# decisionforce/CoPO

Hardware: AMD Instinct MI355X
Metric: agent-env-steps/sec (sim+learn), Intersection 40-agent (higher is better)
Workload: dtype f32; 1 GPU; CoPO Intersection, 40 agent slots x 256 scenes per GPU, fp32 (BASELINE configs[1]); rollout_steps=8, sgd_minibatch_size_per_rank=512, num_sgd_iter=5, lcf_num_iters=5, parallelism=dp1, hip_graphs=True, policy_init=reference population copo_inter (tests/golden, weights as data)

## Files before the change

copo_amd/_capi.py:

```python
import ctypes as C
import os

_HERE = os.path.dirname(os.path.abspath(__file__))
LIB_PATH = os.path.join(_HERE, "lib", "libcopo_hip.so")
try:
    from . import _libsel as _sel
    if getattr(_sel, "PATH", None):
        LIB_PATH = _sel.PATH
except ImportError:
    pass

from ._abi import *

LCF_STATS_DOUBLES = 8 + 6 * 2048

F_ACTED, F_DONE, F_ARRIVE, F_CRASH, F_OUT, F_MAXSTEP, F_SPAWNED, F_ENV_RESET = (1 << i for i in range(8))
I_VELOCITY, I_STEERING, I_ACCELERATION, I_STEP_REWARD, I_COST, I_EPISODE_LENGTH, I_EPISODE_REWARD, \
    I_ROUTE_COMPLETION = range(8)

ERR_NAMES = {0: "COPO_OK", -1: "COPO_ERR_NULL", -2: "COPO_ERR_DIM", -3: "COPO_ERR_DEVICE", -4: "COPO_ERR_STATE",
             -5: "COPO_ERR_CONFIG"}


class CopoError(RuntimeError):
# ... 11 lines not shown
    _fields_ = [
        ("mb", C.c_int32), ("hidden", C.c_int32), ("act_dim", C.c_int32), ("n_value_heads", C.c_int32),
        ("pack_width", C.c_int32), ("col_actions", C.c_int32), ("col_logp", C.c_int32), ("col_dist", C.c_int32),
        ("col_adv", C.c_int32), ("col_meta_adv", C.c_int32), ("col_vpred", C.c_int32 * 3), ("col_vtarget", C.c_int32 * 3),
        ("use_kl", C.c_int32), ("old_value_loss", C.c_int32), ("operand_dtype", C.c_int32), ("reserved0", C.c_int32),
        ("clip_param", C.c_float), ("vf_clip_param", C.c_float), ("vf_loss_coeff", C.c_float), ("entropy_coeff", C.c_float),
        ("lr", C.c_float), ("beta1", C.c_float), ("beta2", C.c_float), ("eps", C.c_float),
        ("pol", NetLayout), ("val", NetLayout * 3), ("n_params", C.c_int64),
    ]


HEAD_PPO, HEAD_META_NEW, HEAD_META_OLD = 0, 1, 2
OPERAND_F32, OPERAND_BF16 = 0, 1
PPO_STATS = 8
META_DOT_PARTIALS = 8192

_SIGS = {
    "copo_ppo_workspace_floats": (C.c_int64, [C.POINTER(PpoCfg)]),
    "copo_ppo_fused_step_f32": (C.c_int, [C.POINTER(PpoCfg)] + [C.c_void_p] * 14 + [C.c_int32, C.c_int32, C.c_void_p,
                                                                                   C.c_int32, C.c_void_p, C.c_void_p]),
    "copo_gather_rows_f32": (C.c_int, [C.POINTER(C.c_void_p), C.POINTER(C.c_void_p), C.POINTER(C.c_int32), C.c_int32, C.c_void_p,
                                       C.c_int64, C.c_void_p]),
    "copo_pack_columns_f32": (C.c_int, [C.POINTER(C.c_void_p), C.POINTER(C.c_int32), C.c_int32, C.c_int64, C.c_void_p, C.c_void_p]),
    "copo_dp_workspace_bytes": (C.c_int64, [C.POINTER(PpoCfg), C.c_int32]),
    "copo_ppo_fused_step_dp_f32": (C.c_int, [C.POINTER(PpoCfg)] + [C.c_void_p] * 13 + [C.c_void_p, C.c_int32, C.c_void_p,
                                                                                      C.POINTER(C.c_void_p), C.c_int32, C.c_int32, C.c_void_p]),
    "copo_dp_status": (C.c_int, [C.c_void_p, C.POINTER(PpoCfg), C.c_int32, C.c_void_p]),
    "copo_transpose_weights_f32": (C.c_int, [C.POINTER(PpoCfg), C.c_void_p, C.c_void_p, C.c_void_p]),
    "copo_mlp_forward_f32": (C.c_int, [C.POINTER(PpoCfg)] + [C.c_void_p] * 4 + [C.c_int64, C.c_int32, C.c_int32] +
                             [C.c_void_p] * 7),
# ... 20 lines not shown
    "copo_fault_obs": (C.c_int, [C.c_void_p] * 2 + [C.c_int32] * 5 + [C.c_void_p] * 2 + [C.c_int32] * 2 + [C.c_void_p] * 2 + [C.c_int32, C.c_void_p,
                                 C.c_uint64, C.c_void_p]),
    "copo_fault_act": (C.c_int, [C.c_void_p] * 3 + [C.c_int32] * 2 + [C.c_void_p] * 2 + [C.c_int32] * 2 + [C.c_void_p] * 2 + [C.c_int32, C.c_void_p,
                                 C.c_uint64, C.c_void_p]),
    "copo_adam_step_f32": (C.c_int, [C.POINTER(PpoCfg)] + [C.c_void_p] * 4 + [C.c_int64] + [C.c_void_p] * 5),
    "copo_meta_grads_f32": (C.c_int, [C.POINTER(PpoCfg)] + [C.c_void_p] * 15),
    "copo_meta_lcf_f64": (C.c_int, [C.c_void_p, C.c_int32, C.c_int32, C.c_int32] + [C.c_void_p] * 4 + [C.c_int32] +
                          [C.c_void_p] * 5),
    "copo_meta_finish_f64": (C.c_int, [C.c_void_p, C.c_void_p, C.c_int64, C.c_void_p, C.c_void_p, C.c_void_p, C.c_void_p, C.c_double,
                                       C.c_void_p, C.c_void_p, C.c_void_p, C.c_void_p, C.c_int32, C.c_void_p]),
    "copo_meta_step_f64": (C.c_int, [C.POINTER(PpoCfg)] + [C.c_void_p] * 13 + [C.c_int32, C.c_int32] + [C.c_void_p] * 5 +
                           [C.c_double, C.c_void_p, C.c_void_p, C.c_int32, C.c_void_p]),
    "copo_episode_metrics": (C.c_int, [C.c_void_p, C.c_void_p, C.c_void_p, C.c_int64, C.c_void_p, C.c_void_p]),
    "copo_plan_epoch": (C.c_int, [C.c_void_p, C.c_void_p, C.c_void_p, C.c_int64, C.c_int32, C.c_int32, C.c_void_p, C.c_int32] +
                        [C.c_void_p] * 5),
    "copo_meta_fold_len": (C.c_int64, [C.POINTER(PpoCfg)]),
    "copo_meta_batch_workspace_floats": (C.c_int64, [C.POINTER(PpoCfg), C.c_int32]),
    "copo_meta_batch_grads_f32": (C.c_int, [C.POINTER(PpoCfg)] + [C.c_void_p] * 8 + [C.c_int32, C.c_int64, C.c_int32] + [C.c_void_p] * 4),
    "copo_meta_batch_dot_f64": (C.c_int, [C.c_void_p, C.c_int64, C.c_int32, C.c_void_p, C.c_void_p, C.c_void_p, C.c_void_p]),
    "copo_meta_rows_workspace_floats": (C.c_int64, [C.POINTER(PpoCfg), C.c_int64]),
    "copo_meta_rows_f32": (C.c_int, [C.POINTER(PpoCfg)] + [C.c_void_p] * 4 + [C.c_int64] + [C.c_void_p] * 3),
    "copo_meta_batch_wgrads_f32": (C.c_int, [C.POINTER(PpoCfg)] + [C.c_void_p] * 5 + [C.c_int64] + [C.c_void_p] * 2 +
                                   [C.c_int32, C.c_int64, C.c_int32] + [C.c_void_p] * 4),
    "copo_meta_rowstat_f32": (C.c_int, [C.POINTER(PpoCfg)] + [C.c_void_p] * 4 + [C.c_int64, C.c_int32, C.c_void_p, C.c_void_p]),
    "copo_meta_batch_lcf_f64": (C.c_int, [C.c_void_p, C.c_int32, C.c_int32, C.c_int32, C.c_void_p, C.c_void_p, C.c_int32] +
                                [C.c_void_p] * 3 + [C.c_int32, C.c_int32] + [C.c_void_p] * 5 + [C.c_double, C.c_void_p, C.c_int32, C.c_int32, C.c_int32, C.c_void_p, C.c_void_p]),
    "copo_version": (C.c_int, []),
    "copo_build_info": (C.c_char_p, []),
    "copo_last_error": (C.c_char_p, []),
    "copo_sim_create": (C.c_int, [C.POINTER(SimCfg), C.c_int, C.POINTER(C.c_void_p)]),
# ... 82 lines not shown
    "copo_recorder_count": (C.c_int, [C.c_void_p, C.POINTER(C.c_int64), C.c_void_p]),
    "copo_recorder_read": (C.c_int, [C.c_void_p, C.c_int32, C.c_int32, C.c_void_p, C.c_void_p]),
    "copo_recorder_episodes": (C.c_int, [C.c_void_p, C.c_void_p, C.c_void_p]),
    "copo_recorder_clear": (C.c_int, [C.c_void_p, C.c_void_p]),
    "copo_recorder_reset": (C.c_int, [C.c_void_p, C.c_void_p]),
    "copo_recorder_destroy": (C.c_int, [C.c_void_p]),
    "copo_neighbours_f32": (C.c_int, [C.c_void_p, C.c_void_p, C.c_void_p, C.c_int32, C.c_int32, C.c_int32, C.c_float,
                                      C.c_float, C.c_void_p, C.c_void_p, C.c_void_p, C.c_void_p, C.c_void_p,
                                      C.c_void_p, C.c_void_p]),
    "copo_gae3_f32": (C.c_int, [C.c_void_p, C.c_void_p, C.c_void_p, C.c_int32, C.c_int32, C.c_int32,
                                C.POINTER(C.c_double), C.c_double, C.c_void_p, C.c_void_p, C.c_void_p]),
    "copo_cc_fuse_mf_f32": (C.c_int, [C.c_void_p] * 5 + [C.c_int32] * 6 + [C.c_void_p, C.c_void_p]),
    "copo_cc_fuse_concat_f32": (C.c_int, [C.c_void_p] * 5 + [C.c_int32] * 7 + [C.c_void_p, C.c_void_p]),
    "copo_lcf_mix_partial_f32": (C.c_int, [C.c_void_p] * 5 + [C.c_int64, C.c_void_p, C.c_void_p, C.c_void_p]),
    "copo_lcf_mix_apply_f32": (C.c_int, [C.c_void_p] * 3 + [C.c_int64, C.c_void_p, C.c_void_p, C.c_void_p, C.c_void_p]),
    "copo_peer_workspace_bytes": (C.c_int64, [C.c_int64, C.c_int32]),
    "copo_peer_alloc": (C.c_int, [C.c_int64, C.POINTER(C.c_void_p)]),
    "copo_peer_free": (C.c_int, [C.c_void_p]),
    "copo_ipc_export": (C.c_int, [C.c_void_p, C.c_char_p]),
    "copo_ipc_open": (C.c_int, [C.c_char_p, C.POINTER(C.c_void_p)]),
    "copo_ipc_close": (C.c_int, [C.c_void_p]),
    "copo_peer_allreduce_sum_f32": (C.c_int, [C.POINTER(C.c_void_p), C.c_int64, C.c_int32, C.c_int32, C.c_void_p]),
    "copo_peer_status": (C.c_int, [C.c_void_p, C.c_int64, C.c_int32, C.c_void_p]),
    "copo_debug_peer_allreduce_all_ranks": (C.c_int, [C.POINTER(C.c_void_p), C.c_int64, C.c_int32, C.c_void_p]),
    "copo_debug_rowpass_stamps": (C.c_int, [C.c_void_p]),
    "copo_debug_wg_times": (C.c_int, [C.c_void_p]),
    "copo_debug_learner_plan": (C.c_int, [C.POINTER(PpoCfg), C.c_int32, C.c_int32, C.c_int64] + [C.c_int32] * 5 + [C.c_void_p, C.c_int32]),
    "copo_debug_learner_kernel": (C.c_char_p, [C.c_int32, C.POINTER(C.c_int32), C.POINTER(C.c_int32)]),
}

# ... 40 lines not shown
```

copo_amd/csrc/capi.hip:

```cpp
#include <cstdarg>
#include <cstdio>
#include <cstring>
#include <new>
#include <algorithm>
#include <vector>
#include <cmath>

#include "capi_common.h"
#include "seat_common.h"
#include "fault_common.h"

using namespace copo;

static thread_local char g_err[512] = "";

int copo::fail(int code, const char* fmt, ...) {
    va_list ap;
    va_start(ap, fmt);
    vsnprintf(g_err, sizeof(g_err), fmt, ap);
    va_end(ap);
    return code;
}

extern "C" int copo_version(void) { return COPO_ABI_VERSION; }
// ... 503 lines not shown
extern "C" int copo_lcf_mix_partial_f32(const float* adv, const float* nei_adv, const float* glob_adv, const float* lcf,
                                        const uint8_t* valid, int64_t B, float* mixed, double* stats, void* stream) {
    if (!adv || !nei_adv || !glob_adv || !lcf || !mixed || !stats)
        return fail(COPO_ERR_NULL, "copo_lcf_mix_partial_f32: NULL argument");
    if (B < 0) return fail(COPO_ERR_DIM, "copo_lcf_mix_partial_f32: B=%lld", (long long)B);
    HIP_TRY(launch_lcf_mix_partial(adv, nei_adv, glob_adv, lcf, valid, B, mixed, stats, static_cast<hipStream_t>(stream)));
    return COPO_OK;
}

extern "C" int copo_lcf_mix_apply_f32(const float* mixed, const float* glob_adv, const uint8_t* valid, int64_t B,
                                      const double* stats, float* norm_adv, float* glob_adv_std, void* stream) {
    if (!mixed || !glob_adv || !stats || !norm_adv || !glob_adv_std)
        return fail(COPO_ERR_NULL, "copo_lcf_mix_apply_f32: NULL argument");
    if (B < 0) return fail(COPO_ERR_DIM, "copo_lcf_mix_apply_f32: B=%lld", (long long)B);
    if (B == 0) return COPO_OK;
    HIP_TRY(launch_lcf_mix_apply(mixed, glob_adv, valid, B, stats, norm_adv, glob_adv_std, static_cast<hipStream_t>(stream)));
    return COPO_OK;
}
```

copo_amd/csrc/learn_kernels.hip:

```cpp
#include <string.h>

#include "sim_common.h"

namespace copo {

struct Gae3Args {
    double gamma[4];
    double lam;
};

__global__ void __launch_bounds__(256) gae3_kernel(const float* __restrict__ rew, const float* __restrict__ val,
                                                   const uint8_t* __restrict__ flags, int T, int M, int heads,
                                                   Gae3Args a, float* __restrict__ adv, float* __restrict__ tgt) {
    const long long gid = (long long)blockIdx.x * blockDim.x + threadIdx.x;
    if (gid >= (long long)heads * M) return;
    const int hd = (int)(gid / M), m = (int)(gid - (long long)hd * M);
    const size_t hoff = (size_t)hd * T * M;
    const double g64 = a.gamma[hd];
    const float g32 = (float)g64;
    const double c = g64 * a.lam;
    double acc = 0.0, vnext64 = 0.0;
    float vnext32 = 0.0f;
    bool seg_done = false, in_seg = false;
    for (int t = T - 1; t >= 0; --t) {
// ... 203 lines not shown
    }
}

__global__ void __launch_bounds__(384) lcf_mix_fold_kernel(double* __restrict__ stats, int nblocks) {
    const int k = threadIdx.x >> 6, lane = threadIdx.x & 63;
    double s = 0.0;
    for (int b = lane; b < nblocks; b += 64) s += stats[8 + 6 * b + k];
    s = wave_sum(s);
    if (lane == 0) stats[k] = s;
}

__global__ void __launch_bounds__(256) lcf_mix_apply_kernel(const float* __restrict__ mixed,
                                                            const float* __restrict__ glob,
                                                            const uint8_t* __restrict__ valid, long long B, int vec,
                                                            const double* __restrict__ stats,
                                                            float* __restrict__ norm_adv, float* __restrict__ glob_std) {
    const double m0 = stats[1] / stats[0], v0 = stats[2] / stats[0] - m0 * m0;
    const double m1 = stats[4] / stats[3], v1 = stats[5] / stats[3] - m1 * m1;
    double s0 = sqrt(v0 > 0 ? v0 : 0), s1 = sqrt(v1 > 0 ? v1 : 0);
    if (s0 < 1e-4) s0 = 1e-4;
    if (s1 < 1e-4) s1 = 1e-4;
    const long long stride = (long long)gridDim.x * blockDim.x * 4;
    for (long long i = ((long long)blockIdx.x * blockDim.x + threadIdx.x) * 4; i < B; i += stride) {
        float vm[4], vg[4], o0[4], o1[4];
        lcf_ld4(mixed, i, B, vec, vm);
        lcf_ld4(glob, i, B, vec, vg);
#pragma unroll
        for (int u = 0; u < 4; ++u) {
            const bool ok = i + u < B && (!valid || valid[i + u < B ? i + u : B - 1]);
            o0[u] = ok ? (float)(((double)vm[u] - m0) / s0) : 0.0f;
            o1[u] = ok ? (float)(((double)vg[u] - m1) / s1) : 0.0f;
        }
// ... 11 lines not shown
static int lcf_aligned(const void* a, const void* b, const void* c, const void* d) {
    return ((reinterpret_cast<uintptr_t>(a) | reinterpret_cast<uintptr_t>(b) | reinterpret_cast<uintptr_t>(c) |
             reinterpret_cast<uintptr_t>(d)) & 15) == 0;
}

hipError_t launch_lcf_mix_partial(const float* adv, const float* nei_adv, const float* glob_adv, const float* lcf,
                                  const uint8_t* valid, int64_t B, float* mixed, double* stats, hipStream_t stream) {
    const int vec = lcf_aligned(adv, nei_adv, glob_adv, lcf) && ((reinterpret_cast<uintptr_t>(mixed) & 15) == 0);
    hipLaunchKernelGGL(lcf_mix_partial_kernel, dim3(kLcfBlocks), dim3(256), 0, stream, adv, nei_adv, glob_adv, lcf,
                       valid, (long long)B, vec, mixed, stats);
    hipLaunchKernelGGL(lcf_mix_fold_kernel, dim3(1), dim3(384), 0, stream, stats, kLcfBlocks);
    return hipGetLastError();
}

hipError_t launch_lcf_mix_apply(const float* mixed, const float* glob_adv, const uint8_t* valid, int64_t B,
                                const double* stats, float* norm_adv, float* glob_std, hipStream_t stream) {
    const int vec = lcf_aligned(mixed, glob_adv, norm_adv, glob_std);
    int grid = (int)((B + 1023) / 1024);
    if (grid > 4096) grid = 4096;
    if (grid < 1) grid = 1;
    hipLaunchKernelGGL(lcf_mix_apply_kernel, dim3(grid), dim3(256), 0, stream, mixed, glob_adv, valid, (long long)B, vec,
                       stats, norm_adv, glob_std);
    return hipGetLastError();
}

__global__ void __launch_bounds__(1024) episode_metrics_kernel(const uint8_t* flags, const float* info, const int32_t* nbr_cnt,
                                                               int64_t R, double* out) {
    __shared__ double red[16][15];
    double s[15];
#pragma unroll
    for (int k = 0; k < 15; ++k) s[k] = 0.0;
    for (int64_t i = threadIdx.x; i < R; i += blockDim.x) {
        const unsigned f = flags[i];
        if (!(f & COPO_F_ACTED)) continue;
        const float* q = info + i * COPO_INFO_DIM;
        s[8] += 1.0;
#pragma unroll
// ... 48 lines not shown

struct PlanArgs {
    const int64_t* valid_idx;
    const int64_t* perm;
    uint32_t key[4];
    uint32_t half;
    int64_t B_local;
    int32_t n_mb, mb, world;
    int64_t B_all[16];
    int64_t* rows;
    float* w;
    float* denom;
    int64_t* k_index;
};

__global__ void __launch_bounds__(256) plan_epoch_kernel(PlanArgs a) {
    const int64_t i = (int64_t)blockIdx.x * 256 + threadIdx.x;
    const int64_t total = (int64_t)a.n_mb * a.mb;
    if (i == 0 && a.k_index) a.k_index[0] = 0;
    if (i < a.n_mb) {
        double d = 0.0;
        for (int r = 0; r < a.world; ++r) d += (double)(a.B_all[r] / a.n_mb + (i < a.B_all[r] % a.n_mb ? 1 : 0));
        a.denom[i] = (float)(d > 1.0 ? d : 1.0);
    }
    if (i >= total) return;
    const int k = (int)(i / a.mb), j = (int)(i - (int64_t)k * a.mb);
    const int64_t q = a.B_local / a.n_mb, r = a.B_local % a.n_mb;
    const int64_t start = k * q + (k < r ? k : r), size = q + (k < r ? 1 : 0);
    const bool in = j < size && a.B_local > 0;
    int64_t row = 0;
    if (in) {
        int64_t pos = start + j;
        pos = pos < a.B_local ? pos : a.B_local - 1;
        row = a.valid_idx[a.perm ? a.perm[pos] : (int64_t)feistel_perm((uint32_t)pos, (uint32_t)a.B_local, a.half, a.key)];
    }
    a.rows[i] = row;
    a.w[i] = in ? 1.0f : 0.0f;
}

hipError_t launch_plan_epoch(const PlanArgs& a, hipStream_t s) {
    const int64_t total = (int64_t)a.n_mb * a.mb;
    hipLaunchKernelGGL(plan_epoch_kernel, dim3((unsigned)((total + 255) / 256)), dim3(256), 0, s, a);
    return hipGetLastError();
}

struct GatherArgs {
    const float* src[COPO_GATHER_MAX_SRC];
    float* dst[COPO_GATHER_MAX_SRC];
    int32_t width[COPO_GATHER_MAX_SRC];
    int32_t n_src;
    const int64_t* rows;
    int64_t n_rows;
};
__global__ void __launch_bounds__(256) gather_rows_kernel(GatherArgs a) {
    const int lane = threadIdx.x & 63;
    const int64_t r = (int64_t)blockIdx.x * 4 + (threadIdx.x >> 6);
    if (r >= a.n_rows) return;
    const int64_t sr = a.rows[r];
// ... 84 lines not shown
extern "C" int copo_plan_epoch(const int64_t* valid_idx, const int64_t* perm, const uint32_t* key4_host, int64_t B_local,
                               int32_t n_mb, int32_t mb, const int64_t* B_all_host, int32_t world, int64_t* rows, float* w,
                               float* denom, int64_t* mb_index, void* stream) {
    if (!rows || !w || !denom || !B_all_host || (B_local > 0 && (!valid_idx || (!perm && !key4_host)))) return COPO_ERR_NULL;
    if (B_local < 0 || B_local > 0x7fffffffLL || n_mb < 1 || mb < 1 || world < 1 || world > 16) return COPO_ERR_DIM;
    copo::PlanArgs a;
    int bits = 1;
    while ((1LL << bits) < B_local) ++bits;
    a.half = (uint32_t)((bits + 1) / 2);
    for (int k = 0; k < 4; ++k) a.key[k] = key4_host ? key4_host[k] : 0u;
    a.valid_idx = valid_idx; a.perm = perm; a.B_local = B_local; a.n_mb = n_mb; a.mb = mb; a.world = world;
    for (int r = 0; r < 16; ++r) a.B_all[r] = r < world ? B_all_host[r] : 0;
    a.rows = rows; a.w = w; a.denom = denom; a.k_index = mb_index;
    return copo::launch_plan_epoch(a, static_cast<hipStream_t>(stream)) == hipSuccess ? COPO_OK : COPO_ERR_DEVICE;
}
```

copo_amd/csrc/sim_common.h:

```cpp
#pragma once
#include <hip/hip_runtime.h>
#include <stdint.h>

#include "../../include/copo_hip.h"
#include "sim_math.h"

#define COPO_SIM_MAX_BLOCK 1024

namespace copo {

enum : int { ST_EMPTY = 0, ST_ALIVE = 1, ST_WRECK = 2 };
enum : uint32_t { RNG_ROUTE = 1, RNG_LCF1 = 2, RNG_LCF2 = 3, RNG_SPAWN = 4, RNG_PERM = 16 };

struct SimParams {
    int32_t E, N, O, K, num_lasers, enable_lcf, horizon, delay_done, respawn_cooldown, substeps;
    int32_t n_routes, n_spawns, n_safe, n_lines;
    int32_t n_spaces;
    int32_t chunk;
    int32_t nbr_chunk;
    int32_t chunk_one_wave;
    int32_t stage_tables;
    int32_t pack_scenes;
    int32_t seg_rows;
    int32_t side_lasers, lane_lasers, navi_dim, toll_dim, toll_min_steps;
// ... 44 lines not shown
hipError_t launch_sim_step_packed(const SimParams& p, const SimParams* p_dev, const float* act, const StepOut& out, int S, hipStream_t stream);
hipError_t launch_neighbours(const float* pos, const uint8_t* present, const float* rew, const SimParams& p,
                             const StepOut& out, hipStream_t stream);

hipError_t launch_gae3(const float* rew, const float* val, const uint8_t* flags, int T, int M, int heads,
                       const double* gamma_host, double lam, float* adv, float* tgt, hipStream_t stream);
hipError_t launch_cc_fuse_mf(const float* obs, const float* act, const uint8_t* flags, const int32_t* nbr_idx,
                             const int32_t* cnt, int R, int N, int O, int A, int K, int counterfactual, float* cc,
                             hipStream_t stream);
hipError_t launch_cc_fuse_concat(const float* obs, const float* act, const uint8_t* flags, const int32_t* nbr_idx,
                                 const int32_t* cnt, int R, int N, int O, int A, int K, int num_neighbours,
                                 int counterfactual, float* cc, hipStream_t stream);
hipError_t launch_lcf_mix_partial(const float* adv, const float* nei_adv, const float* glob_adv, const float* lcf,
                                  const uint8_t* valid, int64_t B, float* mixed, double* stats, hipStream_t stream);
hipError_t launch_lcf_mix_apply(const float* mixed, const float* glob_adv, const uint8_t* valid, int64_t B,
                                const double* stats, float* norm_adv, float* glob_std, hipStream_t stream);

}
```

copo_amd/ops.py:

```python
import ctypes as C

import torch

from . import _capi

F_ACTED, F_DONE = _capi.F_ACTED, _capi.F_DONE


def _chk(*tensors):
    for t in tensors:
        if t is None:
            continue
        if not t.is_cuda:
            raise RuntimeError("copo_amd.ops: expected a CUDA tensor (the HIP path has no CPU fallback)")
        if not t.is_contiguous():
            raise RuntimeError("copo_amd.ops: tensors must be contiguous")


def neighbours(pos, present, rew=None, K=8, radius=40.0, mf_distance=10.0):
    _chk(pos, present, rew)
    E, N = pos.shape[0], pos.shape[1]
    dev = pos.device
    o = dict(nbr_idx=torch.empty(E, N, K, dtype=torch.int32, device=dev),
             nbr_cnt=torch.empty(E, N, dtype=torch.int32, device=dev),
# ... 49 lines not shown


def lcf_mix_partial(adv, nei_adv, glob_adv, lcf, valid, mixed, stats):
    _chk(adv, nei_adv, glob_adv, lcf, valid, mixed, stats)
    assert stats.dtype == torch.float64 and stats.numel() >= _capi.LCF_STATS_DOUBLES
    _capi.check(_capi.lib.copo_lcf_mix_partial_f32(adv.data_ptr(), nei_adv.data_ptr(), glob_adv.data_ptr(),
                                                   lcf.data_ptr(), _capi.ptr(valid), adv.numel(), mixed.data_ptr(),
                                                   stats.data_ptr(), _capi.current_stream()))


def lcf_mix_apply(mixed, glob_adv, valid, stats, norm_adv, glob_std):
    _chk(mixed, glob_adv, valid, stats, norm_adv, glob_std)
    _capi.check(_capi.lib.copo_lcf_mix_apply_f32(mixed.data_ptr(), glob_adv.data_ptr(), _capi.ptr(valid), mixed.numel(),
                                                 stats.data_ptr(), norm_adv.data_ptr(), glob_std.data_ptr(),
                                                 _capi.current_stream()))
```

copo_amd/torch_copo/algo_copo.py:

```python
import math
import os

import numpy as np
import torch
import torch.nn as nn

from copo_amd import dist as D
from copo_amd.engine import (LEARNER_STATS_KEY, NUM_AGENT_STEPS_SAMPLED, NUM_ENV_STEPS_SAMPLED, Postprocessing,
                             SampleBatch, build_mlp, reduce_mean_valid_fn)
from copo_amd.hostread import HostRead, PendingResult
from copo_amd.torch_copo.algo_ccppo import (CENTRALIZED_CRITIC_OBS, COUNTERFACTUAL, CCModel, CCPPOConfig, CCPPOPolicy,
                                            CCPPOTrainer)
from copo_amd.torch_copo.algo_ippo import clipped_value_loss
from copo_amd.trainer import GraphedCallable

NEI_REWARDS = "nei_rewards"
NEI_VALUES = "nei_values"
NEI_ADVANTAGE = "nei_advantage"
NEI_TARGET = "nei_target"
LCF_LR = "lcf_lr"
GLOBAL_VALUES = "global_values"
GLOBAL_REWARDS = "global_rewards"
GLOBAL_ADVANTAGES = "global_advantages"
GLOBAL_TARGET = "global_target"
# ... 519 lines not shown

    def _wants_row_store(self, mb, num_iters):
        rs = self._row_sources
        nb_batch = int(self.config.get("meta_batch_size", 32)) if self.fused is not None else 0
        return nb_batch > 0 and bool(self.config.get("meta_row_store", True)) and num_iters > 1 \
            and mb == rs["mb"] and int(rs["max_rows"]) <= int(self.config.get("meta_row_store_max_rows", 1 << 20))

    def meta_rows_early(self, mb, num_iters):
        if self.fused is None or self._meta_bufs is None or self._meta_bufs["mb"] != mb or not self._wants_row_store(mb, num_iters) \
                or int(self.config.get("meta_batch_size", 32)) <= 0:
            return False
        self.fused.meta_rows(self._row_sources)
        self._rows_early = True
        return True

    def run_meta(self, valid_idx, B_local, B_all, mb, num_iters, defer=False, extra=None):
        rs = self._row_sources
        dev = self.device
        max_mb = max(rs["max_mb"], 1) if mb == rs["mb"] else max(1, math.ceil(rs["max_mb"] * rs["mb"] / mb))
        n_pol = sum(p.numel() for p in self.model.policy_parameters())
        if self._meta_bufs is None or self._meta_bufs["mb"] != mb or self._meta_bufs["max_mb"] != max_mb:
            self._meta_bufs = dict(
                mb=mb, max_mb=max_mb, rows_all=torch.zeros(max_mb, mb, dtype=torch.int64, device=dev),
                w_all=torch.zeros(max_mb, mb, dtype=torch.float32, device=dev),
                denom_all=torch.ones(max_mb, dtype=torch.float32, device=dev),
                k=torch.zeros(1, dtype=torch.int64, device=dev),
                eps_all=torch.zeros(max_mb, mb, dtype=torch.float64, device=dev),
                flat=torch.zeros(2 * n_pol + 3, dtype=torch.float64, device=dev),
                stats_a=torch.zeros(4, dtype=torch.float64, device=dev),
                stats=torch.zeros(len(self.META_KEYS), dtype=torch.float64, device=dev), n_pol=n_pol)
# ... 8 lines not shown
                self._meta_bufs.update(
                    g_both=g_both, g_new=g_both[:nflat], g_old=g_both[n_pol:], tail=torch.zeros(4, dtype=torch.float64, device=dev),
                    dot_partials=torch.zeros(8192, dtype=torch.float64, device=dev),
                    stats_new=torch.zeros(8, device=dev), stats_old=torch.zeros(8, device=dev),
                    col_adv=cols[Postprocessing.ADVANTAGES], col_nei_adv=cols[NEI_ADVANTAGE],
                    gv=torch.zeros(max_mb, dtype=torch.float64, device=dev),
                    stats_k=torch.zeros(max_mb, 2, 8, dtype=torch.float32, device=dev))
            self._meta = None
        if self._meta is None:
            if D.is_dist():
                self._meta = (GraphedCallable(self._meta_step_a, self.use_graphs),
                              GraphedCallable(self._meta_step_b, self.use_graphs))
            else:
                self._meta = GraphedCallable(self._meta_step_local, self.use_graphs)
        mbuf = self._meta_bufs
        mbuf["stats"].zero_()
        steps = 0
        nb_batch = int(self.config.get("meta_batch_size", 32)) if self.fused is not None else 0
        self._meta_row_store = self._wants_row_store(mb, num_iters)
        early, self._rows_early = self._rows_early, False
        if self._meta_row_store and not early:
            self.fused.meta_rows(rs)
        perms = self.draw_perms(num_iters, B_local)
        chunked = self._meta_row_store and self._meta_per_chunk()
        if chunked:
            if mbuf.get("en_cols") is None:
                mbuf["en_cols"] = torch.tensor([mbuf["col_adv"], mbuf["col_nei_adv"]], dtype=torch.int64, device=dev)
            mbuf["en_src"] = rs["pack"].index_select(1, mbuf["en_cols"])
            if mbuf.get("sets") is None:
                keys = ("rows_all", "w_all", "denom_all", "eps_all")
                mbuf["sets"] = [{k: mbuf[k] for k in keys}, {k: torch.zeros_like(mbuf[k]) for k in keys}]
                mbuf["sets"][1]["denom_all"].fill_(1.0)
                mbuf["pass_no"], mbuf["pass_done"] = 0, [None, None]
        for it in range(num_iters):
            if chunked:
                q = mbuf["pass_no"] & 1
                if mbuf["pass_done"][q] is not None:
                    torch.cuda.current_stream().wait_event(mbuf["pass_done"][q])
                mbuf.update(mbuf["sets"][q])
            n_mb = self.plan_epoch(valid_idx, B_local, B_all, mb, bufs=mbuf, perm=None if perms is None else perms[it])
            mbuf["eps_all"].normal_()
            if nb_batch > 0:
                self._run_meta_batched(n_mb, nb_batch)
# ... 101 lines not shown

    def get_default_policy_class(self, config):
        assert config["framework"] == "torch"
        return CoPOPolicy

    def coordinated_advantage(self, batch, valid):
        from copo_amd import ops
        pol = self.policy
        dev = pol.device
        n = batch[SampleBatch.FLAGS].numel()
        if self._mix_ws is None or self._mix_ws["n"] != n:
            self._mix_ws = dict(n=n, stats=ops.lcf_stats_workspace(dev), mixed=torch.empty(n, device=dev),
                                norm=torch.empty(n, device=dev), gstd=torch.empty(n, device=dev),
                                valid=torch.empty(n, dtype=torch.uint8, device=dev))
        ws = self._mix_ws
        ws["valid"].copy_(valid)
        adv = batch[Postprocessing.ADVANTAGES].reshape(-1)
        nei = batch[NEI_ADVANTAGE].reshape(-1)
        glob = batch[GLOBAL_ADVANTAGES].reshape(-1).contiguous()
        lcf = batch["step_lcf"].reshape(-1)
        ops.lcf_mix_partial(adv.contiguous(), nei.contiguous(), glob, lcf.contiguous(), ws["valid"], ws["mixed"], ws["stats"])
        D.all_reduce_sum_(ws["stats"][:6])
        ops.lcf_mix_apply(ws["mixed"], glob, ws["valid"], ws["stats"], ws["norm"], ws["gstd"])
        s = ws["stats"]
        mean = s[1] / s[0]
        std = torch.clamp(torch.sqrt(torch.clamp(s[2] / s[0] - mean * mean, min=0.0)), min=1e-4)
        pol._raw_lcf_adv_mean.copy_(mean)
        pol._raw_lcf_adv_std.copy_(std)
        shape = batch[SampleBatch.FLAGS].shape
        batch["raw_normalized_advantages"] = ws["mixed"].view(shape)
        batch["normalized_advantages"] = ws["norm"].view(shape)
        batch[GLOBAL_ADVANTAGES] = ws["gstd"].view(shape)

    def training_step(self):
        import time
        cfg, pol = self.config, self.policy
        batch = self.collect()
        valid, idx, B = self.valid_rows(batch)
        B_all = D.all_gather_int(B, pol.device)
        self._counters[NUM_AGENT_STEPS_SAMPLED] += sum(B_all)
        self._counters[NUM_ENV_STEPS_SAMPLED] += self.sampler.T * self.sampler.E * D.world_size()
        self.coordinated_advantage(batch, valid)
        t0 = time.perf_counter()
        mb = int(cfg["sgd_minibatch_size"])
        pol.prepare_sgd(batch, batch[SampleBatch.FLAGS].numel(), mb)
        lcf_mb = int(cfg["lcf_sgd_minibatch_size"] or cfg["sgd_minibatch_size"])
        pending = pol.run_sgd(idx, B, B_all, mb, int(cfg["num_sgd_iter"]), defer=True)
        if not D.is_dist():
            pending.start()
            pol.meta_rows_early(lcf_mb, int(cfg["lcf_num_iters"]))
        stats = pending()
        self._timers["learn_time_ms"] = (time.perf_counter() - t0) * 1e3
        t0 = time.perf_counter()
        sums = self._episode.rider()
        extra = {} if sums is None else {"episode_sums": sums}
        pending_meta = pol.run_meta(idx, B, B_all, lcf_mb, int(cfg["lcf_num_iters"]), defer=True, extra=extra)
        lcf_parameters = pol.model.lcf_parameters.detach().clone()

        def _update_lcf_dev(w_id, w):
            def _update_lcf_1(pi, pi_id):
# ... 40 lines not shown
```

copo_amd/trainer.py:

```python
import ctypes as C
import math
import os
import time
from collections import defaultdict

import numpy as np
import torch

from . import dist as D
from .engine import (LEARNER_STATS_KEY, NUM_AGENT_STEPS_SAMPLED, NUM_ENV_STEPS_SAMPLED, Postprocessing, SampleBatch,
                     TorchDiagGaussian)
from .hostread import HostRead, PendingResult, PinnedBuffer

F_ACTED, F_DONE, F_ARRIVE, F_CRASH, F_OUT, F_MAXSTEP, F_SPAWNED, F_ENV_RESET = (1 << i for i in range(8))


def resolve_device(cfg_device=None):
    if cfg_device is not None:
        return torch.device(cfg_device)
    if torch.cuda.is_available():
        return torch.device("cuda", D.env_world()[1])
    return torch.device("cpu")


# ... 376 lines not shown
        w = (j[None, :] < size[:, None])
        if B_local > 0:
            rows = perm[torch.clamp(pos, max=B_local - 1)]
        else:
            rows = torch.zeros(n_mb, mb, dtype=torch.int64, device=dev)
        rs["rows_all"][:n_mb].copy_(torch.where(w, rows, torch.zeros_like(rows)))
        rs["w_all"][:n_mb].copy_(w.to(torch.float32))
        denom = np.zeros(n_mb, np.float64)
        for Br in B_all:
            qq, rr = divmod(Br, n_mb)
            denom += qq + (np.arange(n_mb) < rr)
        rs["denom_all"][:n_mb].copy_(torch.as_tensor(np.maximum(denom, 1.0), dtype=torch.float32))
        rs["k"].zero_()
        return n_mb

    def fused_adv_keys(self):
        return Postprocessing.ADVANTAGES, None

    _tile = None
    _dp_mode = None

    _rs_step = None
    _sgd_chain = _sgd_chain_long = None
    _gather_ok = None
    _dp_fault_injected = False

    def _fused_local(self):
        rs = self._rs_step if self._rs_step is not None else self._row_sources
        if self._dp_mode == "tile":
            self.fused.step_dp(rs, self._tile, stats=self.fused.stats)
        else:
            self.fused.step(rs, stats=self.fused.stats)

    SGD_CHAIN = int(os.environ.get("COPO_SGD_CHAIN", "16"))

    def _fused_local_chain(self):
        for _ in range(self.SGD_CHAIN):
            self._fused_local()

    SGD_CHAIN_LONG = int(os.environ.get("COPO_SGD_CHAIN_LONG", "0"))
# ... 80 lines not shown
    def _rccl_epoch(self, n_mb):
        grads, apply, apply_then_grads = self._sgd
        for k in range(n_mb):
            (grads if k == 0 else apply_then_grads)()
            self._grad_all_reduce()
        apply()

    def _fused_epochs(self, valid_idx, B_local, B_all, mb, num_epochs, perms):
        fz, rs0 = self.fused, self._row_sources
        local = self._dp_mode == "tile" or not D.is_dist()
        n_mb_ep = max(1, math.ceil(max(B_all) / mb))
        if self._gather_ok is None:
            self._gather_ok = bool(self.config.get("gather_epoch_rows", True) and fz.gather_epoch_ok(rs0))
        if local and self.use_graphs and self._gather_ok and self.config.get("plan_all_epochs", True) \
                and num_epochs * n_mb_ep <= int(rs0["rows_all"].shape[0]):
            for ep in range(num_epochs):
                o = ep * n_mb_ep
                self.plan_epoch(valid_idx, B_local, B_all, mb, perm=None if perms is None else perms[ep],
                                bufs=dict(rows_all=rs0["rows_all"][o:], w_all=rs0["w_all"][o:], denom_all=rs0["denom_all"][o:], k=rs0["k"]))
            total = num_epochs * n_mb_ep
            self._rs_step = fz.gather_epoch(rs0, total)
            self._walk(total)
            return total
        steps = 0
        for ep in range(num_epochs):
            n_mb = self.plan_epoch(valid_idx, B_local, B_all, mb, perm=None if perms is None else perms[ep])
            if not local:
                self._rccl_epoch(n_mb)
            else:
                if self._gather_ok:
                    self._rs_step = fz.gather_epoch(rs0, n_mb)
                self._walk(n_mb)
            steps += n_mb
        return steps
# ... 41 lines not shown

    def _read_stats(self, keys, sums, steps, defer):
        D.all_reduce_sum_(sums)
        means = sums / max(1, steps)
        pending = PendingResult(HostRead([("means", means)], pin=self._stats_pinned),
                                lambda parts: self.learner_stats(keys, parts["means"], steps))
        return pending if defer else pending()

    def run_sgd_fused(self, valid_idx, B_local, B_all, mb, num_epochs, defer=False):
        fz = self.fused
        assert mb == fz.cfg.mb, "fused learner was built for minibatch %d" % fz.cfg.mb
        perms = None
        while True:
            self._build_fused_sgd()
            snap = self._tile_snapshot()
            fz.stats.zero_()
            fz.sync_mirror()
            if perms is None:
                perms = self.draw_perms(num_epochs, B_local)
            steps = self._fused_epochs(valid_idx, B_local, B_all, mb, num_epochs, perms)
            self.num_grad_updates += steps
            if self._tile is None or self._tile_agreed(snap):
                return self._read_stats(self.FUSED_STAT_KEYS, fz.stats, steps, defer)

    def run_sgd(self, valid_idx, B_local, B_all, mb, num_epochs, defer=False):
        if self.fused is not None:
            return self.run_sgd_fused(valid_idx, B_local, B_all, mb, num_epochs, defer=defer)
        self._ensure_flat_grads()
        rs = self._row_sources
        if self._sgd is None:
            if D.is_dist():
# ... 482 lines not shown
```

include/copo_hip.h:

```cpp
#ifndef COPO_HIP_H
#define COPO_HIP_H

#include <stdint.h>

#ifdef __cplusplus
extern "C" {
#endif

#define COPO_ABI_VERSION 8

#define COPO_OK 0
#define COPO_ERR_NULL (-1)
#define COPO_ERR_DIM (-2)
#define COPO_ERR_DEVICE (-3)
#define COPO_ERR_STATE (-4)
#define COPO_ERR_CONFIG (-5)

#define COPO_MAX_AGENTS 64
#define COPO_MAX_SEGS 16
#define COPO_SEG_STRIDE 16
#define COPO_MAX_LASERS 256
#define COPO_MAX_BOXES 16
#define COPO_BOX_STRIDE 6
#define COPO_MAX_SPAWNS 256
// ... 335 lines not shown

int copo_gae3_f32(const float* rew, const float* val, const uint8_t* flags, int32_t T, int32_t M, int32_t heads,
                  const double* gamma, double lam, float* adv, float* tgt, void* stream);

int copo_cc_fuse_mf_f32(const float* obs, const float* act, const uint8_t* flags, const int32_t* nbr_idx,
                        const int32_t* cnt, int32_t R, int32_t N, int32_t O, int32_t A, int32_t K,
                        int32_t counterfactual, float* cc_obs, void* stream);
int copo_cc_fuse_concat_f32(const float* obs, const float* act, const uint8_t* flags, const int32_t* nbr_idx,
                            const int32_t* cnt, int32_t R, int32_t N, int32_t O, int32_t A, int32_t K,
                            int32_t num_neighbours, int32_t counterfactual, float* cc_obs, void* stream);

int copo_lcf_mix_partial_f32(const float* adv, const float* nei_adv, const float* glob_adv, const float* lcf,
                             const uint8_t* valid, int64_t B, float* mixed, double* stats, void* stream);
int copo_lcf_mix_apply_f32(const float* mixed, const float* glob_adv, const uint8_t* valid, int64_t B,
                           const double* stats, float* norm_adv, float* glob_adv_std, void* stream);

int copo_episode_metrics(const uint8_t* flags, const float* info, const int32_t* nbr_cnt, int64_t n_rows, double* out15,
                         void* stream);

#define COPO_GATHER_MAX_SRC 4
#define COPO_PACK_MAX_COLS 24
int copo_gather_rows_f32(const float* const* srcs, float* const* dsts, const int32_t* widths, int32_t n_src, const int64_t* rows,
                         int64_t n_rows, void* stream);
int copo_pack_columns_f32(const float* const* cols, const int32_t* widths, int32_t n_cols, int64_t n_rows, float* pack,
                          void* stream);

int copo_plan_epoch(const int64_t* valid_idx, const int64_t* perm, const uint32_t* key4_host, int64_t B_local, int32_t n_mb,
                    int32_t mb, const int64_t* B_all_host, int32_t world, int64_t* rows, float* w, float* denom,
                    int64_t* mb_index, void* stream);

typedef struct copo_net_layout {
    int64_t w1, b1, w2, b2, w3, b3;
    int32_t in_dim, out_dim;
} copo_net_layout;

#define COPO_HEAD_PPO 0
#define COPO_HEAD_META_NEW 1
#define COPO_HEAD_META_OLD 2
#define COPO_PPO_MAX_MB 1024
#define COPO_META_BATCH_MAX 256
#define COPO_META_DOT_PARTIALS 8192
#define COPO_PPO_MAX_KSPLIT 4
#define COPO_OPERAND_F32 0
#define COPO_OPERAND_BF16 1
// ... 138 lines not shown
```

Measured before the change: 2.981 million agent-steps/s.

## Batch epoch planning, iteration prologue and LCF mix finish into fewer launches

Replaces the per-epoch plan_epoch loop with one 2D-grid kernel that plans all epochs at once, using per-epoch keys passed by value. Adds a prologue kernel that zeroes the PPO and meta stats buffers and extracts the two advantage columns in one launch, replacing separate zero_ and index_select calls. Folds the raw LCF mean and std computation into the mix-apply kernel and avoids copying the valid mask when it is already usable. The aim is fewer small kernel launches and less Python glue per training iteration, at the cost of new state flags (_stats_cleared, prologue_done) that must stay in sync across stages.

```diff
diff --git a/copo_amd/_capi.py b/copo_amd/_capi.py
--- a/copo_amd/_capi.py
+++ b/copo_amd/_capi.py
@@ -49,6 +49,7 @@
 OPERAND_F32, OPERAND_BF16 = 0, 1
 PPO_STATS = 8
 META_DOT_PARTIALS = 8192
+PLAN_MAX_EPOCHS = 64
 
 _SIGS = {
     "copo_ppo_workspace_floats": (C.c_int64, [C.POINTER(PpoCfg)]),
@@ -99,6 +100,10 @@
     "copo_episode_metrics": (C.c_int, [C.c_void_p, C.c_void_p, C.c_void_p, C.c_int64, C.c_void_p, C.c_void_p]),
     "copo_plan_epoch": (C.c_int, [C.c_void_p, C.c_void_p, C.c_void_p, C.c_int64, C.c_int32, C.c_int32, C.c_void_p, C.c_int32] +
                         [C.c_void_p] * 5),
+    "copo_plan_epochs": (C.c_int, [C.c_void_p, C.c_void_p, C.c_void_p, C.c_int32, C.c_int64, C.c_int32, C.c_int32, C.c_void_p, C.c_int32] +
+                         [C.c_void_p] * 5),
+    "copo_iteration_prologue": (C.c_int, [C.c_void_p, C.c_int32, C.c_void_p, C.c_int32, C.c_void_p, C.c_int64, C.c_int32, C.c_void_p,
+                                          C.c_void_p, C.c_void_p]),
     "copo_meta_fold_len": (C.c_int64, [C.POINTER(PpoCfg)]),
     "copo_meta_batch_workspace_floats": (C.c_int64, [C.POINTER(PpoCfg), C.c_int32]),
     "copo_meta_batch_grads_f32": (C.c_int, [C.POINTER(PpoCfg)] + [C.c_void_p] * 8 + [C.c_int32, C.c_int64, C.c_int32] + [C.c_void_p] * 4),
@@ -211,6 +216,7 @@
     "copo_cc_fuse_concat_f32": (C.c_int, [C.c_void_p] * 5 + [C.c_int32] * 7 + [C.c_void_p, C.c_void_p]),
     "copo_lcf_mix_partial_f32": (C.c_int, [C.c_void_p] * 5 + [C.c_int64, C.c_void_p, C.c_void_p, C.c_void_p]),
     "copo_lcf_mix_apply_f32": (C.c_int, [C.c_void_p] * 3 + [C.c_int64, C.c_void_p, C.c_void_p, C.c_void_p, C.c_void_p]),
+    "copo_lcf_mix_finish": (C.c_int, [C.c_void_p] * 3 + [C.c_int64] + [C.c_void_p] * 6),
     "copo_peer_workspace_bytes": (C.c_int64, [C.c_int64, C.c_int32]),
     "copo_peer_alloc": (C.c_int, [C.c_int64, C.POINTER(C.c_void_p)]),
     "copo_peer_free": (C.c_int, [C.c_void_p]),
diff --git a/copo_amd/csrc/capi.hip b/copo_amd/csrc/capi.hip
--- a/copo_amd/csrc/capi.hip
+++ b/copo_amd/csrc/capi.hip
@@ -541,6 +541,15 @@
         return fail(COPO_ERR_NULL, "copo_lcf_mix_apply_f32: NULL argument");
     if (B < 0) return fail(COPO_ERR_DIM, "copo_lcf_mix_apply_f32: B=%lld", (long long)B);
     if (B == 0) return COPO_OK;
-    HIP_TRY(launch_lcf_mix_apply(mixed, glob_adv, valid, B, stats, norm_adv, glob_adv_std, static_cast<hipStream_t>(stream)));
-    return COPO_OK;
-}
+    HIP_TRY(launch_lcf_mix_apply(mixed, glob_adv, valid, B, stats, norm_adv, glob_adv_std, nullptr, nullptr, static_cast<hipStream_t>(stream)));
+    return COPO_OK;
+}
+
+extern "C" int copo_lcf_mix_finish(const float* mixed, const float* glob_adv, const uint8_t* valid, int64_t B, const double* stats,
+                                   float* norm_adv, float* glob_adv_std, double* raw_mean, double* raw_std, void* stream) {
+    if (!stats || !raw_mean || !raw_std || (B > 0 && (!mixed || !glob_adv || !norm_adv || !glob_adv_std)))
+        return fail(COPO_ERR_NULL, "copo_lcf_mix_finish: NULL argument");
+    if (B < 0) return fail(COPO_ERR_DIM, "copo_lcf_mix_finish: B=%lld", (long long)B);
+    HIP_TRY(launch_lcf_mix_apply(mixed, glob_adv, valid, B, stats, norm_adv, glob_adv_std, raw_mean, raw_std, static_cast<hipStream_t>(stream)));
+    return COPO_OK;
+}
diff --git a/copo_amd/csrc/learn_kernels.hip b/copo_amd/csrc/learn_kernels.hip
--- a/copo_amd/csrc/learn_kernels.hip
+++ b/copo_amd/csrc/learn_kernels.hip
@@ -241,8 +241,14 @@
                                                             const float* __restrict__ glob,
                                                             const uint8_t* __restrict__ valid, long long B, int vec,
                                                             const double* __restrict__ stats,
-                                                            float* __restrict__ norm_adv, float* __restrict__ glob_std) {
+                                                            float* __restrict__ norm_adv, float* __restrict__ glob_std,
+                                                            double* raw_mean, double* raw_std) {
     const double m0 = stats[1] / stats[0], v0 = stats[2] / stats[0] - m0 * m0;
+    if (raw_mean && blockIdx.x == 0 && threadIdx.x == 0) {
+        const double c = v0 < 0.0 ? 0.0 : v0, sd = sqrt(c);
+        *raw_mean = m0;
+        *raw_std = sd < 1e-4 ? 1e-4 : sd;
+    }
     const double m1 = stats[4] / stats[3], v1 = stats[5] / stats[3] - m1 * m1;
     double s0 = sqrt(v0 > 0 ? v0 : 0), s1 = sqrt(v1 > 0 ? v1 : 0);
     if (s0 < 1e-4) s0 = 1e-4;
@@ -284,13 +290,14 @@
 }
 
 hipError_t launch_lcf_mix_apply(const float* mixed, const float* glob_adv, const uint8_t* valid, int64_t B,
-                                const double* stats, float* norm_adv, float* glob_std, hipStream_t stream) {
+                                const double* stats, float* norm_adv, float* glob_std, double* raw_mean, double* raw_std,
+                                hipStream_t stream) {
     const int vec = lcf_aligned(mixed, glob_adv, norm_adv, glob_std);
     int grid = (int)((B + 1023) / 1024);
     if (grid > 4096) grid = 4096;
     if (grid < 1) grid = 1;
     hipLaunchKernelGGL(lcf_mix_apply_kernel, dim3(grid), dim3(256), 0, stream, mixed, glob_adv, valid, (long long)B, vec,
-                       stats, norm_adv, glob_std);
+                       stats, norm_adv, glob_std, raw_mean, raw_std);
     return hipGetLastError();
 }
 
@@ -369,14 +376,13 @@
     int64_t* k_index;
 };
 
-__global__ void __launch_bounds__(256) plan_epoch_kernel(PlanArgs a) {
-    const int64_t i = (int64_t)blockIdx.x * 256 + threadIdx.x;
+__device__ __forceinline__ void plan_element(const PlanArgs& a, const int64_t* perm, const uint32_t* key, int64_t* rows, float* w,
+                                             float* denom, int64_t i) {
     const int64_t total = (int64_t)a.n_mb * a.mb;
-    if (i == 0 && a.k_index) a.k_index[0] = 0;
     if (i < a.n_mb) {
         double d = 0.0;
         for (int r = 0; r < a.world; ++r) d += (double)(a.B_all[r] / a.n_mb + (i < a.B_all[r] % a.n_mb ? 1 : 0));
-        a.denom[i] = (float)(d > 1.0 ? d : 1.0);
+        denom[i] = (float)(d > 1.0 ? d : 1.0);
     }
     if (i >= total) return;
     const int k = (int)(i / a.mb), j = (int)(i - (int64_t)k * a.mb);
@@ -387,16 +393,53 @@
     if (in) {
         int64_t pos = start + j;
         pos = pos < a.B_local ? pos : a.B_local - 1;
-        row = a.valid_idx[a.perm ? a.perm[pos] : (int64_t)feistel_perm((uint32_t)pos, (uint32_t)a.B_local, a.half, a.key)];
-    }
-    a.rows[i] = row;
-    a.w[i] = in ? 1.0f : 0.0f;
+        row = a.valid_idx[perm ? perm[pos] : (int64_t)feistel_perm((uint32_t)pos, (uint32_t)a.B_local, a.half, key)];
+    }
+    rows[i] = row;
+    w[i] = in ? 1.0f : 0.0f;
+}
+
+__global__ void __launch_bounds__(256) plan_epoch_kernel(PlanArgs a) {
+    const int64_t i = (int64_t)blockIdx.x * 256 + threadIdx.x;
+    if (i == 0 && a.k_index) a.k_index[0] = 0;
+    plan_element(a, a.perm, a.key, a.rows, a.w, a.denom, i);
 }
 
 hipError_t launch_plan_epoch(const PlanArgs& a, hipStream_t s) {
     const int64_t total = (int64_t)a.n_mb * a.mb;
     hipLaunchKernelGGL(plan_epoch_kernel, dim3((unsigned)((total + 255) / 256)), dim3(256), 0, s, a);
     return hipGetLastError();
+}
+
+struct PlanEpochsArgs {
+    PlanArgs p;
+    uint32_t keys[COPO_PLAN_MAX_EPOCHS][4];
+};
+
+__global__ void __launch_bounds__(256) plan_epochs_kernel(PlanEpochsArgs a) {
+    const int64_t i = (int64_t)blockIdx.x * 256 + threadIdx.x;
+    const int64_t e = blockIdx.y, total = (int64_t)a.p.n_mb * a.p.mb;
+    if (i == 0 && e == 0 && a.p.k_index) a.p.k_index[0] = 0;
+    plan_element(a.p, a.p.perm ? a.p.perm + e * a.p.B_local : nullptr, a.keys[e], a.p.rows + e * total, a.p.w + e * total,
+                 a.p.denom + e * a.p.n_mb, i);
+}
+
+hipError_t launch_plan_epochs(const PlanEpochsArgs& a, int n_epochs, hipStream_t s) {
+    const int64_t total = (int64_t)a.p.n_mb * a.p.mb;
+    hipLaunchKernelGGL(plan_epochs_kernel, dim3((unsigned)((total + 255) / 256), (unsigned)n_epochs), dim3(256), 0, s, a);
+    return hipGetLastError();
+}
+
+__global__ void __launch_bounds__(256) iteration_prologue_kernel(float* zero_f32, int n_f32, double* zero_f64, int n_f64,
+                                                                 const float* __restrict__ pack, long long n_rows, int pack_width,
+                                                                 int col0, int col1, float* __restrict__ en_src) {
+    const long long i = (long long)blockIdx.x * 256 + threadIdx.x;
+    if (i < n_f32) zero_f32[i] = 0.0f;
+    if (i < n_f64) zero_f64[i] = 0.0;
+    if (i < 2 * n_rows) {
+        const long long r = i >> 1;
+        en_src[i] = pack[r * pack_width + ((i & 1) ? col1 : col0)];
+    }
 }
 
 struct GatherArgs {
@@ -511,3 +554,47 @@
     a.rows = rows; a.w = w; a.denom = denom; a.k_index = mb_index;
     return copo::launch_plan_epoch(a, static_cast<hipStream_t>(stream)) == hipSuccess ? COPO_OK : COPO_ERR_DEVICE;
 }
+
+static int plan_args(copo::PlanArgs& a, const int64_t* valid_idx, const int64_t* perm, int64_t B_local, int32_t n_mb, int32_t mb,
+                     const int64_t* B_all_host, int32_t world, int64_t* rows, float* w, float* denom, int64_t* mb_index) {
+    if (B_local < 0 || B_local > 0x7fffffffLL || n_mb < 1 || mb < 1 || world < 1 || world > 16) return COPO_ERR_DIM;
+    int bits = 1;
+    while ((1LL << bits) < B_local) ++bits;
+    a.half = (uint32_t)((bits + 1) / 2);
+    a.valid_idx = valid_idx; a.perm = perm; a.B_local = B_local; a.n_mb = n_mb; a.mb = mb; a.world = world;
+    for (int r = 0; r < 16; ++r) a.B_all[r] = r < world ? B_all_host[r] : 0;
+    a.rows = rows; a.w = w; a.denom = denom; a.k_index = mb_index;
+    return COPO_OK;
+}
+
+extern "C" int copo_plan_epochs(const int64_t* valid_idx, const int64_t* perms, const uint32_t* keys_host, int32_t n_epochs,
+                                int64_t B_local, int32_t n_mb, int32_t mb, const int64_t* B_all_host, int32_t world, int64_t* rows,
+                                float* w, float* denom, int64_t* mb_index, void* stream) {
+    if (!rows || !w || !denom || !B_all_host || (B_local > 0 && (!valid_idx || (!perms && !keys_host)))) return COPO_ERR_NULL;
+    if (n_epochs < 1 || n_epochs > COPO_PLAN_MAX_EPOCHS) return COPO_ERR_DIM;
+    copo::PlanEpochsArgs a;
+    memset(&a, 0, sizeof(a));
+    const int rc = plan_args(a.p, valid_idx, perms, B_local, n_mb, mb, B_all_host, world, rows, w, denom, mb_index);
+    if (rc != COPO_OK) return rc;
+    if (keys_host) memcpy(a.keys, keys_host, sizeof(uint32_t) * 4 * (size_t)n_epochs);
+    return copo::launch_plan_epochs(a, n_epochs, static_cast<hipStream_t>(stream)) == hipSuccess ? COPO_OK : COPO_ERR_DEVICE;
+}
+
+extern "C" int copo_iteration_prologue(float* zero_f32, int32_t n_f32, double* zero_f64, int32_t n_f64, const float* pack,
+                                       int64_t n_rows, int32_t pack_width, const int32_t* cols2_host, float* en_src, void* stream) {
+    if ((n_f32 > 0 && !zero_f32) || (n_f64 > 0 && !zero_f64) || (n_rows > 0 && (!pack || !cols2_host || !en_src))) return COPO_ERR_NULL;
+    if (n_f32 < 0 || n_f64 < 0 || n_rows < 0 || n_rows > 0x7fffffffLL) return COPO_ERR_DIM;
+    int c0 = 0, c1 = 0;
+    if (n_rows > 0) {
+        c0 = cols2_host[0]; c1 = cols2_host[1];
+        if (pack_width < 1 || c0 < 0 || c0 >= pack_width || c1 < 0 || c1 >= pack_width) return COPO_ERR_DIM;
+    }
+    int64_t total = 2 * n_rows;
+    if (total < n_f32) total = n_f32;
+    if (total < n_f64) total = n_f64;
+    if (total == 0) return COPO_OK;
+    hipLaunchKernelGGL(copo::iteration_prologue_kernel, dim3((unsigned)((total + 255) / 256)), dim3(256), 0,
+                       static_cast<hipStream_t>(stream), zero_f32, (int)n_f32, zero_f64, (int)n_f64, pack, (long long)n_rows,
+                       (int)pack_width, c0, c1, en_src);
+    return hipGetLastError() == hipSuccess ? COPO_OK : COPO_ERR_DEVICE;
+}
diff --git a/copo_amd/csrc/sim_common.h b/copo_amd/csrc/sim_common.h
--- a/copo_amd/csrc/sim_common.h
+++ b/copo_amd/csrc/sim_common.h
@@ -82,6 +82,7 @@
 hipError_t launch_lcf_mix_partial(const float* adv, const float* nei_adv, const float* glob_adv, const float* lcf,
                                   const uint8_t* valid, int64_t B, float* mixed, double* stats, hipStream_t stream);
 hipError_t launch_lcf_mix_apply(const float* mixed, const float* glob_adv, const uint8_t* valid, int64_t B,
-                                const double* stats, float* norm_adv, float* glob_std, hipStream_t stream);
+                                const double* stats, float* norm_adv, float* glob_std, double* raw_mean, double* raw_std,
+                                hipStream_t stream);
 
 }
diff --git a/copo_amd/ops.py b/copo_amd/ops.py
--- a/copo_amd/ops.py
+++ b/copo_amd/ops.py
@@ -87,3 +87,11 @@
     _capi.check(_capi.lib.copo_lcf_mix_apply_f32(mixed.data_ptr(), glob_adv.data_ptr(), _capi.ptr(valid), mixed.numel(),
                                                  stats.data_ptr(), norm_adv.data_ptr(), glob_std.data_ptr(),
                                                  _capi.current_stream()))
+
+
+def lcf_mix_finish(mixed, glob_adv, valid, stats, norm_adv, glob_std, raw_mean, raw_std):
+    _chk(mixed, glob_adv, valid, stats, norm_adv, glob_std, raw_mean, raw_std)
+    assert stats.dtype == raw_mean.dtype == raw_std.dtype == torch.float64 and raw_mean.numel() == raw_std.numel() == 1
+    _capi.check(_capi.lib.copo_lcf_mix_finish(mixed.data_ptr(), glob_adv.data_ptr(), _capi.ptr(valid), mixed.numel(),
+                                              stats.data_ptr(), norm_adv.data_ptr(), glob_std.data_ptr(), raw_mean.data_ptr(),
+                                              raw_std.data_ptr(), _capi.current_stream()))
diff --git a/copo_amd/torch_copo/algo_copo.py b/copo_amd/torch_copo/algo_copo.py
--- a/copo_amd/torch_copo/algo_copo.py
+++ b/copo_amd/torch_copo/algo_copo.py
@@ -557,6 +557,25 @@
         self._rows_early = True
         return True
 
+    def iteration_prologue(self):
+        fz, mbuf, rs = self.fused, self._meta_bufs, self._row_sources
+        if fz is None or self.device.type != "cuda" or not self.config.get("native_glue", True) or D.is_dist() \
+                or mbuf is None or "col_adv" not in mbuf or rs is None:
+            return False
+        import ctypes as C
+        from copo_amd import _capi
+        pack = rs["pack"]
+        if mbuf.get("en_buf") is None or mbuf["en_buf"].shape[0] != pack.shape[0]:
+            mbuf["en_buf"] = torch.empty(pack.shape[0], 2, dtype=torch.float32, device=self.device)
+        assert pack.is_contiguous() and pack.dtype == torch.float32 and fz.stats.dtype == torch.float32 \
+            and mbuf["stats"].dtype == torch.float64
+        _capi.check(_capi.lib.copo_iteration_prologue(
+            fz.stats.data_ptr(), fz.stats.numel(), mbuf["stats"].data_ptr(), mbuf["stats"].numel(), pack.data_ptr(),
+            int(pack.shape[0]), int(pack.shape[1]), (C.c_int32 * 2)(int(mbuf["col_adv"]), int(mbuf["col_nei_adv"])),
+            mbuf["en_buf"].data_ptr(), _capi.current_stream()))
+        self._stats_cleared = mbuf["prologue_done"] = True
+        return True
+
     def run_meta(self, valid_idx, B_local, B_all, mb, num_iters, defer=False, extra=None):
         rs = self._row_sources
         dev = self.device
@@ -595,7 +614,9 @@
             else:
                 self._meta = GraphedCallable(self._meta_step_local, self.use_graphs)
         mbuf = self._meta_bufs
-        mbuf["stats"].zero_()
+        prologue = mbuf.pop("prologue_done", False)
+        if not prologue:
+            mbuf["stats"].zero_()
         steps = 0
         nb_batch = int(self.config.get("meta_batch_size", 32)) if self.fused is not None else 0
         self._meta_row_store = self._wants_row_store(mb, num_iters)
@@ -607,7 +628,7 @@
         if chunked:
             if mbuf.get("en_cols") is None:
                 mbuf["en_cols"] = torch.tensor([mbuf["col_adv"], mbuf["col_nei_adv"]], dtype=torch.int64, device=dev)
-            mbuf["en_src"] = rs["pack"].index_select(1, mbuf["en_cols"])
+            mbuf["en_src"] = mbuf["en_buf"] if prologue else rs["pack"].index_select(1, mbuf["en_cols"])
             if mbuf.get("sets") is None:
                 keys = ("rows_all", "w_all", "denom_all", "eps_all")
                 mbuf["sets"] = [{k: mbuf[k] for k in keys}, {k: torch.zeros_like(mbuf[k]) for k in keys}]
@@ -739,19 +760,27 @@
                                 norm=torch.empty(n, device=dev), gstd=torch.empty(n, device=dev),
                                 valid=torch.empty(n, dtype=torch.uint8, device=dev))
         ws = self._mix_ws
-        ws["valid"].copy_(valid)
+        native = bool(self.config.get("native_glue", True)) and dev.type == "cuda"
+        if native and valid.dtype in (torch.uint8, torch.bool) and valid.is_contiguous() and valid.numel() == n:
+            mask = valid.reshape(-1).view(torch.uint8)
+        else:
+            ws["valid"].copy_(valid)
+            mask = ws["valid"]
         adv = batch[Postprocessing.ADVANTAGES].reshape(-1)
         nei = batch[NEI_ADVANTAGE].reshape(-1)
         glob = batch[GLOBAL_ADVANTAGES].reshape(-1).contiguous()
         lcf = batch["step_lcf"].reshape(-1)
-        ops.lcf_mix_partial(adv.contiguous(), nei.contiguous(), glob, lcf.contiguous(), ws["valid"], ws["mixed"], ws["stats"])
+        ops.lcf_mix_partial(adv.contiguous(), nei.contiguous(), glob, lcf.contiguous(), mask, ws["mixed"], ws["stats"])
         D.all_reduce_sum_(ws["stats"][:6])
-        ops.lcf_mix_apply(ws["mixed"], glob, ws["valid"], ws["stats"], ws["norm"], ws["gstd"])
-        s = ws["stats"]
-        mean = s[1] / s[0]
-        std = torch.clamp(torch.sqrt(torch.clamp(s[2] / s[0] - mean * mean, min=0.0)), min=1e-4)
-        pol._raw_lcf_adv_mean.copy_(mean)
-        pol._raw_lcf_adv_std.copy_(std)
+        if native:
+            ops.lcf_mix_finish(ws["mixed"], glob, mask, ws["stats"], ws["norm"], ws["gstd"], pol._raw_lcf_adv_mean, pol._raw_lcf_adv_std)
+        else:
+            ops.lcf_mix_apply(ws["mixed"], glob, mask, ws["stats"], ws["norm"], ws["gstd"])
+            s = ws["stats"]
+            mean = s[1] / s[0]
+            std = torch.clamp(torch.sqrt(torch.clamp(s[2] / s[0] - mean * mean, min=0.0)), min=1e-4)
+            pol._raw_lcf_adv_mean.copy_(mean)
+            pol._raw_lcf_adv_std.copy_(std)
         shape = batch[SampleBatch.FLAGS].shape
         batch["raw_normalized_advantages"] = ws["mixed"].view(shape)
         batch["normalized_advantages"] = ws["norm"].view(shape)
@@ -769,6 +798,7 @@
         t0 = time.perf_counter()
         mb = int(cfg["sgd_minibatch_size"])
         pol.prepare_sgd(batch, batch[SampleBatch.FLAGS].numel(), mb)
+        pol.iteration_prologue()
         lcf_mb = int(cfg["lcf_sgd_minibatch_size"] or cfg["sgd_minibatch_size"])
         pending = pol.run_sgd(idx, B, B_all, mb, int(cfg["num_sgd_iter"]), defer=True)
         if not D.is_dist():
diff --git a/copo_amd/trainer.py b/copo_amd/trainer.py
--- a/copo_amd/trainer.py
+++ b/copo_amd/trainer.py
@@ -414,6 +414,27 @@
         rs["k"].zero_()
         return n_mb
 
+    def plan_epochs(self, valid_idx, B_local, B_all, mb, num_epochs, perms=None):
+        from . import _capi
+        if self.device.type != "cuda" or len(B_all) > 16 or perms is not None or not self.config.get("native_glue", True) \
+                or num_epochs > _capi.PLAN_MAX_EPOCHS or (B_local > 0 and self.config.get("shuffle", "feistel") == "randperm"):
+            return False
+        import ctypes as C
+        rs = self._row_sources
+        n_mb = max(1, math.ceil(max(B_all) / mb))
+        keys = None
+        if B_local > 0:
+            words = []
+            for _ in range(num_epochs):
+                words += [int(v) for v in torch.randint(0, 2 ** 31 - 1, (4,)).tolist()]
+            keys = (C.c_uint32 * len(words))(*words)
+        ball = (C.c_int64 * len(B_all))(*[int(b) for b in B_all])
+        _capi.check(_capi.lib.copo_plan_epochs(
+            valid_idx.data_ptr() if B_local > 0 else None, None, keys, int(num_epochs), int(B_local), int(n_mb), int(mb), ball,
+            len(B_all), rs["rows_all"].data_ptr(), rs["w_all"].data_ptr(), rs["denom_all"].data_ptr(), rs["k"].data_ptr(),
+            _capi.current_stream()))
+        return True
+
     def fused_adv_keys(self):
         return Postprocessing.ADVANTAGES, None
 
@@ -424,6 +445,7 @@
     _sgd_chain = _sgd_chain_long = None
     _gather_ok = None
     _dp_fault_injected = False
+    _stats_cleared = False
 
     def _fused_local(self):
         rs = self._rs_step if self._rs_step is not None else self._row_sources
@@ -534,10 +556,11 @@
             self._gather_ok = bool(self.config.get("gather_epoch_rows", True) and fz.gather_epoch_ok(rs0))
         if local and self.use_graphs and self._gather_ok and self.config.get("plan_all_epochs", True) \
                 and num_epochs * n_mb_ep <= int(rs0["rows_all"].shape[0]):
-            for ep in range(num_epochs):
-                o = ep * n_mb_ep
-                self.plan_epoch(valid_idx, B_local, B_all, mb, perm=None if perms is None else perms[ep],
-                                bufs=dict(rows_all=rs0["rows_all"][o:], w_all=rs0["w_all"][o:], denom_all=rs0["denom_all"][o:], k=rs0["k"]))
+            if not self.plan_epochs(valid_idx, B_local, B_all, mb, num_epochs, perms):
+                for ep in range(num_epochs):
+                    o = ep * n_mb_ep
+                    self.plan_epoch(valid_idx, B_local, B_all, mb, perm=None if perms is None else perms[ep],
+                                    bufs=dict(rows_all=rs0["rows_all"][o:], w_all=rs0["w_all"][o:], denom_all=rs0["denom_all"][o:], k=rs0["k"]))
             total = num_epochs * n_mb_ep
             self._rs_step = fz.gather_epoch(rs0, total)
             self._walk(total)
@@ -609,7 +632,10 @@
         while True:
             self._build_fused_sgd()
             snap = self._tile_snapshot()
-            fz.stats.zero_()
+            if self._stats_cleared:
+                self._stats_cleared = False
+            else:
+                fz.stats.zero_()
             fz.sync_mirror()
             if perms is None:
                 perms = self.draw_perms(num_epochs, B_local)
diff --git a/include/copo_hip.h b/include/copo_hip.h
--- a/include/copo_hip.h
+++ b/include/copo_hip.h
@@ -373,6 +373,8 @@
                              const uint8_t* valid, int64_t B, float* mixed, double* stats, void* stream);
 int copo_lcf_mix_apply_f32(const float* mixed, const float* glob_adv, const uint8_t* valid, int64_t B,
                            const double* stats, float* norm_adv, float* glob_adv_std, void* stream);
+int copo_lcf_mix_finish(const float* mixed, const float* glob_adv, const uint8_t* valid, int64_t B, const double* stats,
+                        float* norm_adv, float* glob_adv_std, double* raw_mean, double* raw_std, void* stream);
 
 int copo_episode_metrics(const uint8_t* flags, const float* info, const int32_t* nbr_cnt, int64_t n_rows, double* out15,
                          void* stream);
@@ -387,6 +389,13 @@
 int copo_plan_epoch(const int64_t* valid_idx, const int64_t* perm, const uint32_t* key4_host, int64_t B_local, int32_t n_mb,
                     int32_t mb, const int64_t* B_all_host, int32_t world, int64_t* rows, float* w, float* denom,
                     int64_t* mb_index, void* stream);
+#define COPO_PLAN_MAX_EPOCHS 64
+int copo_plan_epochs(const int64_t* valid_idx, const int64_t* perms, const uint32_t* keys_host, int32_t n_epochs, int64_t B_local,
+                     int32_t n_mb, int32_t mb, const int64_t* B_all_host, int32_t world, int64_t* rows, float* w, float* denom,
+                     int64_t* mb_index, void* stream);
+
+int copo_iteration_prologue(float* zero_f32, int32_t n_f32, double* zero_f64, int32_t n_f64, const float* pack, int64_t n_rows,
+                            int32_t pack_width, const int32_t* cols2_host, float* en_src, void* stream);
 
 typedef struct copo_net_layout {
     int64_t w1, b1, w2, b2, w3, b3;
```

Measured after the change: 2.988 million agent-steps/s, median of 3. About the same (+0.2%).
